# laiviet/ed-gated-gcn

Hardware: AMD Instinct MI355X
Metric: gated_gcn_forward_edges_per_sec (higher is better)
Workload: dtype f32 (fp16 MFMA + block-scaled fp8 correction MFMA, fp32 accumulate)

## Files before the change

### ed-gated-gcn_amd/csrc/capi.hip

```cpp
#include "fused_args.h"
#include <cstdlib>

#include <cstring>

namespace ggcn {

char *error_buffer()
{
    static thread_local char buf[512] = "";
    return buf;
}

int fail(int code, const char *fmt, ...)
{
    va_list ap;
    va_start(ap, fmt);
    vsnprintf(error_buffer(), 512, fmt, ap);
    va_end(ap);
    return code;
}

namespace {
constexpr int kMaxRangeFlagReaders = 16;
struct RangeFlagReaders {
// ... 415 lines not shown
    const char *form = getenv("GGCN_BLOCK_FORM");
    return (block8_shape(B, T, K, F) && !(form && form[0] == '4')) ? 8 : 4;
}

int ggcn_linear_form(int entry, const void *X, int64_t ldx, const void *W, int64_t ldw, const void *Y, int64_t ldy, int64_t M, int K,
                     int F, int precision)
{
    const char *who = "ggcn_linear_form";
    const uintptr_t xa = reinterpret_cast<uintptr_t>(X), ya = reinterpret_cast<uintptr_t>(Y);
    auto split = [&](int x_bytes, bool y_f32) -> int {
        if (linear_split_grid(M, F) > (int64_t)INT32_MAX) return -fail(GGCN_EUNSUPPORTED, "%s: M too large", who);
        return linear_split_form(x_bytes, y_f32, X, ldx, Y, ldy, K, F);
    };
    switch (entry) {
        case GGCN_ENTRY_LINEAR:
            if (int rc = linear_entry_checks(who, !X || !Y, M, K, F, ldx, ldy)) return -rc;
            if (precision == GGCN_PREC_BF16X3 || precision == GGCN_PREC_F16MX8) return split(4, true);
            if (precision != GGCN_PREC_FP32) return -fail(GGCN_EINVAL, "%s: ggcn_linear has no precision %d", who, precision);
            if (!W) return -fail(GGCN_EINVAL, "%s: ggcn_linear(fp32): W is NULL", who);
            if (ldw < F) return -fail(GGCN_EINVAL, "%s: ggcn_linear(fp32): ldw < F", who);
            return linear_fp32_form(X, ldx, W, ldw, K, F);
        case GGCN_ENTRY_LINEAR_H:
            if (precision != GGCN_PREC_BF16X3 && precision != GGCN_PREC_F16MX8 && precision != GGCN_PREC_F16)
                return -fail(GGCN_EUNSUPPORTED, "%s: ggcn_linear_h has no precision %d", who, precision);
            if (int rc = linear_entry_checks(who, !X || !Y, M, K, F, ldx, ldy)) return -rc;
            if (precision != GGCN_PREC_F16) return split(2, false);
            if (linear_split_grid(M, F) > (int64_t)INT32_MAX) return -fail(GGCN_EUNSUPPORTED, "%s: M too large", who);
            return linear_f16_form(X, ldx, K);
        case GGCN_ENTRY_LINEAR_BF16:
        case GGCN_ENTRY_LINEAR_OUT_BF16: {
            const bool out = entry == GGCN_ENTRY_LINEAR_OUT_BF16;
            if (int rc = linear_entry_checks(who, !X || !Y, M, K, F, ldx, ldy)) return -rc;
            if (xa % (out ? 4 : 2) || ya % (out ? 2 : 4)) return -fail(GGCN_EINVAL, "%s: X / Y not aligned to their element size", who);
            return split(out ? 4 : 2, !out);
        }
        case GGCN_ENTRY_LINEAR_SCALED:
            if (!X || !Y) return -fail(GGCN_EINVAL, "%s: null pointer", who);
            if (M <= 0 || K <= 0 || F <= 0 || ldx < K || ldy < F) return -fail(GGCN_EINVAL, "%s: M=%lld K=%d F=%d", who, (long long)M, K, F);
            if (!linear_scaled_takes(static_cast<const float *>(X), ldx, static_cast<const float *>(Y), ldy, K, F))
                return -fail(GGCN_EUNSUPPORTED, "%s: ggcn_linear_scaled needs K %% 32 == 0, F %% 4 == 0 and 16-byte aligned rows", who);
            return split(4, true);
        default:
            return -fail(GGCN_EINVAL, "%s: unknown entry %d", who, entry);
    }
}

int ggcn_lab_block_fused8(const float *X, int64_t ldx, const void *wpack1, const void *wpack12, const void *graph_ops,
                          const void *graph_ops2, const float *bias1, const float *bias_mid, const float *bias2, int B, int T, int K, int F,
                          const float *gate1, const float *gate2, float *x_out, int64_t ld2, float *x1, float *y1, float *pool_out,
                          float *overlap_partial, uint64_t *stamps, ggcn_stream_t stream)
{
    const int flags = (getenv("GGCN_LAB_BLOCK8_ROWMAJOR") ? kBlock8RowMajor : 0) | (getenv("GGCN_LAB_BLOCK8_NODMA") ? kBlock8NoDma : 0) |
                      (getenv("GGCN_LAB_BLOCK8_SAMESLOTS") ? kBlock8SameSlots : 0) |
                      (getenv("GGCN_LAB_BLOCK8_PRIO") ? kBlock8Prio : 0);
    FusedArgs a = {};
    a.X = X; a.ldx = ldx; a.graph_ops = bytes(graph_ops); a.graph_ops2 = bytes(graph_ops2);
    a.stamps = reinterpret_cast<unsigned long long *>(stamps);
    a.B = B; a.T = T; a.K = K; a.F = F; a.n_parts = 2;
    LayerPart &l1 = a.part[0], &l2 = a.part[1];
    l1.wpack = bytes(wpack1); l1.bias = bias1; l1.pool_gate_a = gate1; l1.pool_gate_b = gate2;
    l1.pool_a = x1; l1.pool_b = y1; l1.ov_partial = overlap_partial;
    l2.wpack = bytes(wpack12); l2.bias = bias2; l2.mid = bias_mid; l2.store_gate = gate2; l2.pool_gate_a = gate2;
    l2.out = x_out; l2.ldo = (int)(ld2 < 0 ? -1 : ld2 > (int64_t)INT32_MAX ? (int64_t)INT32_MAX : ld2); l2.pool_a = pool_out;
    return block_fused8("ggcn_lab_block_fused8", a, flags, as_stream(stream));
}

int ggcn_gate_pool_backward_weighted(const float *out, int64_t ldo, const float *store_gate, const float *gate_a, const float *gate_b,
                                     const float *d_out, int64_t ldd, const float *d_pa, const float *d_pb, const void *graph_ops_wt,
                                     const float *inv, int B, int T, int F, float *dH, int64_t ldh, float *dY, int64_t ldy, float *d_sg,
                                     float *d_ga, float *d_gb, float *d_bsum, ggcn_stream_t stream)
{
    return gate_pool_backward_weighted(out, ldo, store_gate, gate_a, gate_b, d_out, ldd, d_pa, d_pb, graph_ops_wt, inv, B, T, F, dH, ldh,
                                       dY, ldy, d_sg, d_ga, d_gb, d_bsum, as_stream(stream));
}

int ggcn_layer_fused_drop(const float *X, int64_t ldx, const void *wpack, const uint32_t *rowmask, const void *graph_ops,
                          const float *bias, int B, int T, int K, int F, const float *store_gate,
                          const float *pool_gate_a, const float *pool_gate_b, float *out, int64_t ldo,
                          float *pool_a, float *pool_b, int precision, float p, uint64_t seed, int sel_store,
                          int sel_a, int sel_b, ggcn_stream_t stream)
{
    const char *who = "ggcn_layer_fused";
    FusedArgs a = {};
    if (int rc = entry_drop_spec("ggcn_layer_fused_drop", p, seed, sel_store, sel_a, sel_b, a.drop)) return rc;
    if (int rc = layer_entry_checks(who, out, ldo, nullptr, nullptr)) return rc;
    a.X = X; a.ldx = ldx; a.rowmask = rowmask; a.graph_ops = bytes(graph_ops);
    a.B = B; a.T = T; a.K = K; a.F = F; a.n_parts = 1;
    LayerPart &l = a.part[0];
    l.wpack = bytes(wpack); l.bias = bias; l.store_gate = store_gate; l.pool_gate_a = pool_gate_a; l.pool_gate_b = pool_gate_b;
    l.out = out; l.ldo = (int)ldo; l.pool_a = pool_a; l.pool_b = pool_b;
    return launch_fused(who, a, precision, as_stream(stream));
}

size_t ggcn_dweight_workspace_bytes(int64_t n_rows, int K, int F, int precision)
{
    return precision == GGCN_PREC_FP32 ? dweight_workspace_bytes(n_rows, K, F) : dweight_bx3_workspace_bytes(n_rows, K, F);
}

int ggcn_dweight(const float *X, int64_t ldx, const float *dH, int64_t ldg, int64_t n_rows, int K, int F,
                 float *dW, int64_t lddw, int precision, void *workspace, ggcn_stream_t stream)
{
    if (precision == GGCN_PREC_FP32)
        return dweight(X, ldx, dH, ldg, n_rows, K, F, dW, lddw, workspace, as_stream(stream));
    if (precision != GGCN_PREC_BF16X3)
        return fail(GGCN_EUNSUPPORTED, "ggcn_dweight: precision %d (gradients need fp32 range: use bf16x3 or fp32)", precision);
    return dweight_bx3(X, ldx, dH, ldg, n_rows, K, F, dW, lddw, workspace, as_stream(stream));
}
// ... 50 lines not shown
```

### ed-gated-gcn_amd/csrc/f16mx8_core.h

```cpp
#pragma once
#include "bf16x3_core.h"

namespace ggcn {
namespace mx8 {

using namespace bx3;

typedef _Float16 f16x8 __attribute__((ext_vector_type(8)));
typedef int i32x8 __attribute__((ext_vector_type(8)));
typedef int i32x4 __attribute__((ext_vector_type(4)));

#ifndef GGCN_WH8_STORED
#define GGCN_WH8_STORED 0
#endif
constexpr int kWh8Bytes = GGCN_WH8_STORED ? 64 * 16 : 0;
constexpr int kOffWl8 = 2 * 1024, kOffWh8 = kOffWl8 + 64 * 16, kOffScales = kOffWh8 + kWh8Bytes;
constexpr int STAGE_PACK_BYTES = kOffScales + 64 * 4;
constexpr int XL_SHIFT = 11;
constexpr int SCALE_XL = 127 - XL_SHIFT, SCALE_XH = 127;

static __device__ unsigned int g_range_flag;
constexpr float kWindow = 448.0f;
constexpr float kHalfMax = 65504.0f;
__device__ __forceinline__ void range_verdict(float amax, float hb_scale = 0.0f, float hb_add = 0.0f, bool window = true)
// ... 38 lines not shown
    typedef float f2 __attribute__((ext_vector_type(2)));
    typedef short s2 __attribute__((ext_vector_type(2)));
    const h2 p0 = __builtin_convertvector(f2{x0, x1}, h2);
    const h2 p1 = __builtin_convertvector(f2{x2, x3}, h2);
    float r0, r1, r2, r3;
    asm("v_fma_mix_f32 %0, %1, -1.0, %2 op_sel_hi:[1,0,0]" : "=v"(r0) : "v"(p0), "v"(x0));
    asm("v_fma_mix_f32 %0, %1, -1.0, %2 op_sel:[1,0,0] op_sel_hi:[1,0,0]" : "=v"(r1) : "v"(p0), "v"(x1));
    asm("v_fma_mix_f32 %0, %1, -1.0, %2 op_sel_hi:[1,0,0]" : "=v"(r2) : "v"(p1), "v"(x2));
    asm("v_fma_mix_f32 %0, %1, -1.0, %2 op_sel:[1,0,0] op_sel_hi:[1,0,0]" : "=v"(r3) : "v"(p1), "v"(x3));
    constexpr float inv = 1.0f / (float)(1 << XL_SHIFT);
    s2 q = __builtin_bit_cast(s2, undef_vgpr());
    q = __builtin_amdgcn_cvt_scalef32_pk_fp8_f32(q, r0, r1, inv, false);
    q = __builtin_amdgcn_cvt_scalef32_pk_fp8_f32(q, r2, r3, inv, true);
    amax = amax3(x2, x3, amax3(x0, x1, amax));
    int h8 = __builtin_amdgcn_cvt_pk_fp8_f32(x0, x1, undef_vgpr(), false);
    h8 = __builtin_amdgcn_cvt_pk_fp8_f32(x2, x3, h8, true);
    Split4 o;
    o.h01 = __builtin_bit_cast(uint32_t, p0);
    o.h23 = __builtin_bit_cast(uint32_t, p1);
    o.l8 = __builtin_bit_cast(int, q);
    o.h8 = h8;
    return o;
}

__device__ __forceinline__ void set_cvt_saturate(bool on) { __builtin_amdgcn_s_setreg(1 | (23 << 6), on ? 1 : 0); }

__device__ __forceinline__ int q_lds_off(int row, int chunk)
{
    return row * ROWB + ((chunk ^ ((row >> 2) & 3) ^ (((row >> 1) & 1) << 1)) << 4);
}

#define GGCN_SB() __builtin_amdgcn_sched_barrier(0)

template <typename AT>
struct BufX {
    const AT *base;
    uint32_t bytes;
    uint32_t off[Geom<AT>::NP];
};
template <typename AT>
__device__ __forceinline__ BufX<AT> make_bufx(const AT *X, int64_t ldx, int64_t base_row, int64_t total_rows,
                                              const int (&rel)[Geom<AT>::NP], int tid)
{
    BufX<AT> b;
    const int64_t left = (total_rows - base_row) * ldx * (int64_t)sizeof(AT);
    b.base = X + base_row * ldx;
    b.bytes = (uint32_t)(left < 0x7fffffff ? left : 0x7fffffff);
#pragma unroll
    for (int i = 0; i < Geom<AT>::NP; ++i)
        b.off[i] = rel[i] < 0 ? 0x80000000u
                              : (uint32_t)(((int64_t)rel[i] * ldx + (tid % Geom<AT>::TPR) * Geom<AT>::EPT) * (int64_t)sizeof(AT));
    return b;
}
template <typename AT, bool AVEC, bool KFULL, bool ZROWS, bool RBLK = false, bool BUF = false, int NB = 4, bool XS = false, int XP = 4, int SLOT0 = 0>
__device__ __forceinline__ void mainloop(const AT *const (&arow)[Geom<AT>::NP], const bool (&avalid)[Geom<AT>::NP],
                                         const char *__restrict__ wpack, int K, int stages_packed, int wm,
                                         int nt0, int n_tiles_total, char *lds, f32x16 (&acc)[4][RN], int rot = 0, int nblk = 4,
                                         float *amax_out = nullptr, const BufX<AT> *bufx = nullptr, float xscale = 1.0f, int pass0 = 0)
{
    static_assert(!BUF || (AVEC && KFULL && sizeof(AT) == 4), "buffer loads: whole 16-byte pieces of fp32 rows");
    static_assert(NB >= 1 && NB <= 4 && (NB == 4 || (sizeof(AT) == 4 && !RBLK)), "NB < 4: fp32 rows (pass i = block i), no run-time count");
    constexpr int NPL0 = Geom<AT>::NP < NB ? Geom<AT>::NP : NB;
    constexpr int NPL = NPL0 < XP ? NPL0 : XP;
    static_assert(XP == 4 || (sizeof(AT) == 4 && NB == 4 && !RBLK), "XP < 4: fp32 rows, whole tiles");
    static_assert(SLOT0 >= 0 && SLOT0 + XP <= 4, "the staging passes sit behind the stage's four row-block slots");
    using G = Geom<AT>;
    constexpr int EPT = G::EPT, NP = G::NP, NQ = EPT / 4;
    static_assert(BK == 32 && NP <= 4 && RN == 2, "the slot schedule below is written for BK = 32, <= 4 passes, RN = 2");
    const int tid = threadIdx.x & (kThreads - 1);
    const int lane = tid & 63;
    const int s_k = (tid % G::TPR) * EPT;

    set_cvt_saturate(true);
    float amax = 0.0f;

    constexpr int kRsrcFlags = 0x00020000;
    __amdgpu_buffer_rsrc_t xr, wr;
    if constexpr (BUF) {
        xr = __builtin_amdgcn_make_buffer_rsrc(const_cast<AT *>(bufx->base), 0, (int)bufx->bytes, kRsrcFlags);
        wr = __builtin_amdgcn_make_buffer_rsrc(const_cast<char *>(wpack), 0, 0x7fffffff, kRsrcFlags);
    }
    float ra[NP][EPT];
    auto load_a_pass = [&](int i, int k0) {
        const int gk = k0 + s_k;
        if constexpr (BUF) {
            const float4 t = __builtin_bit_cast(float4, __builtin_amdgcn_raw_buffer_load_b128(xr, bufx->off[i], k0 * (int)sizeof(AT), 0));
            ra[i][0] = t.x; ra[i][1] = t.y; ra[i][2] = t.z; ra[i][3] = t.w;
        } else if constexpr (AVEC) {
            load16<AT>(arow[i] + ((KFULL || gk < K) ? gk : 0), ra[i]);
        } else {
#pragma unroll
            for (int c = 0; c < EPT; ++c) ra[i][c] = elem_to_float(arow[i][(gk + c < K) ? gk + c : 0]);
        }
    };
    Split4 sp[NQ];
    auto split_pass = [&](int i, int k0) {
        const int gk = k0 + s_k;
#pragma unroll
        for (int q = 0; q < NQ; ++q) {
            float x[4];
#pragma unroll
            for (int c = 0; c < 4; ++c) {
                x[c] = ra[i][4 * q + c];
                if constexpr (!KFULL || ZROWS) {
                    bool in = true;
                    if constexpr (!KFULL) in = gk + 4 * q + c < K;
                    if constexpr (ZROWS && !BUF) in = in && avalid[i];
                    x[c] = in ? x[c] : 0.0f;
                }
                if constexpr (XS) x[c] *= xscale;
            }
            sp[q] = split4(x[0], x[1], x[2], x[3], amax);
        }
    };
    auto write_pass = [&](int buf, int i) {
        char *h_plane = lds + buf * (2 * BM * ROWB);
        char *q_plane = h_plane + BM * ROWB;
        const int row = stage_row<AT>(XP == 4 ? i : i + pass0);
#pragma unroll
        for (int q = 0; q < NQ; ++q) {
            const int kq = s_k + 4 * q;
            *reinterpret_cast<uint2 *>(h_plane + a_lds_off(row, kq >> 3) + (kq & 4) * 2) = make_uint2(sp[q].h01, sp[q].h23);
// ... 57 lines not shown
    auto wh8_of = [&](const f16x8 &f0, const f16x8 &f1, int sc) -> i32x4 {
        typedef _Float16 h2 __attribute__((ext_vector_type(2)));
        typedef short s2 __attribute__((ext_vector_type(2)));
        const float inv = __builtin_bit_cast(float, (sc & 0xff00) << 15);
        i32x4 o;
#pragma unroll
        for (int d = 0; d < 4; ++d) {
            const f16x8 &f = d < 2 ? f0 : f1;
            const int e = (d & 1) * 4;
            s2 q = __builtin_bit_cast(s2, undef_vgpr());
            q = __builtin_amdgcn_cvt_scalef32_pk_fp8_f16(q, h2{f[e], f[e + 1]}, inv, false);
            q = __builtin_amdgcn_cvt_scalef32_pk_fp8_f16(q, h2{f[e + 2], f[e + 3]}, inv, true);
            o[d] = __builtin_bit_cast(int, q);
        }
        return o;
    };

    const int f_row = wm * 128 + (lane & 31);
    const int f_half = lane >> 5;
    const int scale_a = f_half ? SCALE_XH : SCALE_XL;
    auto read_h = [&](int buf, int i, f16x8 (&a)[2]) {
        const char *h_plane = lds + buf * (2 * BM * ROWB);
        const int row = f_row + i * 32;
        a[0] = *reinterpret_cast<const f16x8 *>(h_plane + a_lds_off(row, f_half));
        a[1] = *reinterpret_cast<const f16x8 *>(h_plane + a_lds_off(row, 2 + f_half));
    };
    auto read_q = [&](int buf, int i, i32x8 &a) {
        const char *q_plane = lds + buf * (2 * BM * ROWB) + BM * ROWB;
        const int row = f_row + i * 32;
        const i32x4 lo = *reinterpret_cast<const i32x4 *>(q_plane + q_lds_off(row, f_half));
        const i32x4 hi = *reinterpret_cast<const i32x4 *>(q_plane + q_lds_off(row, 2 + f_half));
        a = __builtin_shufflevector(lo, hi, 0, 1, 2, 3, 4, 5, 6, 7);
    };

#pragma unroll
    for (int i = 0; i < 4; ++i)
#pragma unroll
        for (int j = 0; j < RN; ++j)
#pragma unroll
            for (int r = 0; r < 16; ++r) acc[i][j][r] = 0.0f;

    f16x8 b0[RN], b1[RN];
    i32x4 bq[RN];
    i32x4 bw[RN];
    int sq[RN];
    const int stages = (K + BK - 1) / BK;

    auto kstage = [&](int n) {
        n = n < stages ? n : stages - 1;
        const int s = n + rot;
        return s >= stages ? s - stages : s;
    };
#pragma unroll
    for (int p = 0; p < NPL; ++p) load_a_pass(p, kstage(0) * BK);
    load_bf(kstage(0), b0, b1);
#pragma unroll
    for (int p = 0; p < NPL; ++p) {
        split_pass(p, kstage(0) * BK);
        write_pass(0, p);
    }
#pragma unroll
    for (int p = 0; p < NPL; ++p) load_a_pass(p, kstage(1) * BK);
    __syncthreads();

    auto stage = [&](int st, auto bufc) {
        constexpr int buf = decltype(bufc)::value;
        const int k_next1 = kstage(st + 1) * BK;
        const int ka = kstage(st + 2) * BK;
        f16x8 ah[2][2];
        i32x8 aq[2];
        read_h(buf, 0, ah[0]);
        load_bq(kstage(st), bq, sq);
        if constexpr (GGCN_WH8_STORED) load_wh8(kstage(st), bw);
        GGCN_SB();
#pragma unroll
        for (int i = 0; i < NB; ++i) {
            const bool stages_here = i - SLOT0 >= 0 && i - SLOT0 < NP && i - SLOT0 < XP;
            if (i < NB - 1) read_h(buf, i + 1, ah[(i + 1) & 1]);
            else read_q(buf, 0, aq[0]);
            GGCN_SB();
            if (!RBLK || i < nblk) acc[i][0] = __builtin_amdgcn_mfma_f32_32x32x16_f16(ah[i & 1][0], b0[0], acc[i][0], 0, 0, 0);
            GGCN_SB();
            if (stages_here) split_pass(i - SLOT0, k_next1);
            GGCN_SB();
            if (!RBLK || i < nblk) acc[i][1] = __builtin_amdgcn_mfma_f32_32x32x16_f16(ah[i & 1][0], b0[1], acc[i][1], 0, 0, 0);
            GGCN_SB();
            if (stages_here) write_pass(buf ^ 1, i - SLOT0);
            GGCN_SB();
            if (!RBLK || i < nblk) acc[i][0] = __builtin_amdgcn_mfma_f32_32x32x16_f16(ah[i & 1][1], b1[0], acc[i][0], 0, 0, 0);
            GGCN_SB();
            if (stages_here) load_a_pass(i - SLOT0, ka);
            GGCN_SB();
            if (!RBLK || i < nblk) acc[i][1] = __builtin_amdgcn_mfma_f32_32x32x16_f16(ah[i & 1][1], b1[1], acc[i][1], 0, 0, 0);
            GGCN_SB();
        }
        i32x8 bm[RN];
#pragma unroll
        for (int j = 0; j < RN; ++j) {
            i32x4 w;
            if constexpr (GGCN_WH8_STORED) w = bw[j];
            else w = wh8_of(b0[j], b1[j], sq[j]);
            bm[j] = i32x8{w[0], w[1], w[2], w[3], bq[j][0], bq[j][1], bq[j][2], bq[j][3]};
        }
        GGCN_SB();
#pragma unroll
        for (int i = 0; i < NB; ++i) {
            if (i < NB - 1) read_q(buf, i + 1, aq[(i + 1) & 1]);
// ... 25 lines not shown
```

### ed-gated-gcn_amd/csrc/fused_args.h

```cpp
#pragma once
#include "common.h"
#include "dropout_hash.h"

namespace ggcn {

struct LayerPart {
    const char *wpack;
    const float *bias;
    const float *mid;
    const float *pre;
    const float *store_gate;
    const float *pool_gate_a;
    const float *pool_gate_b;
    float *out;
    float *pool_a, *pool_b;
    float *ov_partial;
    int ldo;
};

struct FusedArgs {
    const float *X;
    int64_t ldx;
    const uint32_t *rowmask;
    const char *graph_ops;
    const char *graph_ops2;
    const float *ov_in;
    float *ov_out;
    int B, T, K, F;
    int g_tiles, n_wg, n_parts, k_steps;
    LayerPart part[2];
    DropSpec drop;
    unsigned long long *stamps;
    const __bf16 *Xb;
};

inline bool vector_row_stores(const FusedArgs &a, const LayerPart &lp)
{
    return (a.F % 4 == 0) && (lp.ldo % 4 == 0) && aligned16(lp.out) && (int64_t)a.T * lp.ldo * 4 < ((int64_t)1 << 31);
}

int fused_part_checks(const char *who, const FusedArgs &a, bool &vst);

int launch_fused(const char *who, FusedArgs &a, int precision, hipStream_t st, bool weighted_block = false);

int launch_fused_weighted_wide(const char *who, FusedArgs &a, int precision, hipStream_t st);

enum BlockKind { kBlockBinary, kBlockWeighted, kBlockBf16 };
int launch_block(const char *who, FusedArgs &a, BlockKind kind, int precision, hipStream_t st);

constexpr int kBlock8RowMajor = 1, kBlock8NoDma = 2, kBlock8SameSlots = 4, kBlock8Prio = 8;
bool block8_shape(int B, int T, int K, int F);
bool block8_takes(const FusedArgs &a);
int block_fused8(const char *who, FusedArgs &a, int flags, hipStream_t st);

}
```

### ed-gated-gcn_amd/csrc/fused_block8.hip

```cpp
#include "fused_common.h"

#include <cstdlib>

namespace ggcn {
namespace {

constexpr int kB8Threads = 512;
constexpr int kB8Lds = kLdsBytes + 2 * kEpiLdsBytes;

__device__ __forceinline__ bool getenv_slot_same(const FusedArgs &a) { return (a.k_steps & 0x20000000) != 0; }

template <int BASE>
__device__ __forceinline__ float staged_mid_max(const char *lds, bool dma, int lane)
{
    if (dma) {
        const float4 m4 = *reinterpret_cast<const float4 *>(lds + EpiLds<BASE>::kBias + BN * 4 + lane * 16);
        float mm = fmaxf(fmaxf(fabsf(m4.x), fabsf(m4.y)), fmaxf(fabsf(m4.z), fabsf(m4.w)));
#pragma unroll
        for (int d = 32; d >= 1; d >>= 1) mm = fmaxf(mm, __shfl_xor(mm, d));
        return mm;
    }
    const float4 mm = *reinterpret_cast<const float4 *>(lds + EpiLds<BASE>::kMidMax);
    return fmaxf(fmaxf(mm.x, mm.y), fmaxf(mm.z, mm.w));
}

template <bool FULLT, bool VST>
__global__ __launch_bounds__(kB8Threads, 1) void block_fused8_kernel(const FusedArgs a)
{
    extern __shared__ __attribute__((aligned(16))) char lds[];
    const int B = a.B, T = a.T, K = a.K, F = a.F;
    int n_wgi, g_tile;
    if (a.n_parts == 2) {
        const int xcd = blockIdx.x & 7, qb = blockIdx.x >> 3;
        const int total = a.g_tiles * a.n_wg, per_xcd = (total + 7) >> 3;
        const int w = xcd * per_xcd + qb;
        if (qb >= per_xcd || w >= total) return;
        n_wgi = w / a.g_tiles;
        g_tile = w - n_wgi * a.g_tiles;
    } else {
        if (!tile_of_block(blockIdx.x, a.g_tiles, a.n_wg, g_tile, n_wgi)) return;
    }

    const int tid8 = threadIdx.x;
    const unsigned long long t_start = a.stamps ? __builtin_amdgcn_s_memrealtime() : 0;
    const int group = __builtin_amdgcn_readfirstlane(tid8 >> 8);
    const int tid = tid8 & 255;
    const int wave = __builtin_amdgcn_readfirstlane(tid >> 6);
    const LayerPart &lp = a.part[group];
    const int gt0 = g_tile * 4, g0 = gt0;
    const int n_tiles_total = (F + NT - 1) / NT;
    const int nt0 = n_wgi * (BN / NT) + wave * RN;

    constexpr int NP = Geom<float>::NP;
    const float *arow[NP];
    bool avalid[NP];
    int rel[NP];
#pragma unroll
    for (int i = 0; i < NP; ++i) {
        const int row = stage_row<float>(i < 2 ? i + 2 * group : 0);
        const int g = gt0 + (row >> 5), r = row & 31;
        avalid[i] = i < 2 && (g < B) && (FULLT || r < T);
        arow[i] = a.X;
        rel[i] = avalid[i] ? (row >> 5) * T + (row & 31) : -1;
    }
    const bool dma = (a.n_wg * BN == F) && (gt0 + 4 <= B) && a.ov_in == nullptr && a.ov_out == nullptr && (a.k_steps & 0x40000000) != 0;
    const int k_steps = a.k_steps & 0x0fffffff;
    if (dma) {
        if (group == 0) stage_epilogue_operands_dma<kLdsBytes>(a, lp, g0, n_wgi, lds, tid);
        else stage_epilogue_operands_dma<kLdsBytes + kEpiLdsBytes>(a, lp, g0, n_wgi, lds, tid);
    } else {
        if (group == 0) stage_epilogue_operands<kLdsBytes>(a, lp, g0, n_wgi, lds, tid);
        else stage_epilogue_operands<kLdsBytes + kEpiLdsBytes>(a, lp, g0, n_wgi, lds, tid);
    }

    f32x16 acc[4][RN];
    float amax;
    const int64_t pack_bytes = (int64_t)n_tiles_total * (k_steps / 2) * mx8::STAGE_PACK_BYTES;
    const float bw1 = *reinterpret_cast<const float *>(a.part[0].wpack + pack_bytes);
    const float bw12 = *reinterpret_cast<const float *>(a.part[1].wpack + pack_bytes);
    const unsigned long long t_loop0 = a.stamps ? __builtin_amdgcn_s_memrealtime() : 0;
    mx8::BufX<float> bx = mx8::make_bufx<float>(a.X, a.ldx, (int64_t)gt0 * T, (int64_t)B * T, rel, tid);
    if (group == 1 && (a.k_steps & 0x10000000) != 0) __builtin_amdgcn_s_setprio(1);
    if (group == 0 || getenv_slot_same(a))
        mx8::mainloop<float, true, true, !FULLT, false, true, 4, false, 2, 0>(arow, avalid, lp.wpack, K, k_steps / 2, 0, nt0, n_tiles_total, lds, acc, 0, 4,
                                                                               &amax, &bx, 1.0f, 2 * group);
    else
        mx8::mainloop<float, true, true, !FULLT, false, true, 4, false, 2, 2>(arow, avalid, lp.wpack, K, k_steps / 2, 0, nt0, n_tiles_total, lds, acc, 0, 4,
                                                                               &amax, &bx, 1.0f, 2 * group);
    unsigned long long t_loop1 = 0;
    if (a.stamps) { asm volatile("" :: "v"(acc[3][RN - 1][15])); t_loop1 = __builtin_amdgcn_s_memrealtime(); }
    mx8::range_verdict(amax, bw12, staged_mid_max<kLdsBytes + kEpiLdsBytes>(lds, dma, tid & 63), true);
    mx8::range_verdict(amax, bw1, 0.0f, false);
    if (group == 0) {
        epilogue<1, FULLT, VST, false, false, kLdsBytes>(a, lp, acc, g0, nt0, n_tiles_total, lds, tid);
    } else {
        if (lp.out) epilogue<1, FULLT, VST, true, true, kLdsBytes + kEpiLdsBytes>(a, lp, acc, g0, nt0, n_tiles_total, lds, tid);
        else epilogue<1, FULLT, VST, true, false, kLdsBytes + kEpiLdsBytes>(a, lp, acc, g0, nt0, n_tiles_total, lds, tid);
    }
    if (a.stamps && tid == 0) {
        unsigned long long *o = a.stamps + ((size_t)blockIdx.x * 2 + group) * 4;
        o[0] = t_start; o[1] = t_loop0; o[2] = t_loop1; o[3] = __builtin_amdgcn_s_memrealtime();
    }
}

}

int device_cu_count()
{
    static int cus = 0;
    if (cus == 0) {
        int dev = 0, n = 0;
        if (hipGetDevice(&dev) != hipSuccess || hipDeviceGetAttribute(&n, hipDeviceAttributeMultiprocessorCount, dev) != hipSuccess || n <= 0) n = 256;
        cus = n;
    }
    return cus;
}
bool block8_shape(int B, int T, int K, int F)
{
    if (B <= 0 || T > 32 || T <= 0 || F <= 0 || K <= 0 || F % BN != 0 || K % BK != 0) return false;
    const int64_t total = (int64_t)((B + 3) / 4) * (F / BN), cus = device_cu_count();
    return total >= 6 * cus || (total >= 3 * cus && total % cus == 0);
}
static bool block8_fast_x(const FusedArgs &a)
{
    return (a.K % BK == 0) && (a.ldx % 4 == 0) && aligned16(a.X) && (int64_t)a.ldx * 4 * 257 < ((int64_t)1 << 31);
}
static bool block8_dma_aligned(const FusedArgs &a)
{
    const LayerPart &l1 = a.part[0], &l2 = a.part[1];
    return aligned16(l1.pool_gate_a) && aligned16(l2.store_gate) && aligned16(l1.bias) && aligned16(l2.bias) && aligned16(l2.mid) &&
           aligned16(a.graph_ops) && aligned16(a.graph_ops2);
}
bool block8_takes(const FusedArgs &a)
{
    const LayerPart &l1 = a.part[0], &l2 = a.part[1];
    if (!block8_shape(a.B, a.T, a.K, a.F)) return false;
    if (!a.X || !l1.wpack || !l2.wpack || a.ldx < a.K || !aligned16(l1.wpack) || !aligned16(l2.wpack) || (l2.out && l2.ldo < a.F)) return false;
    if (!block8_fast_x(a)) return false;
    if (!a.graph_ops || !a.graph_ops2 || !l1.pool_gate_a || !l2.store_gate || !l2.mid) return false;
    if (!block8_dma_aligned(a)) return false;
    if (l2.out && !vector_row_stores(a, l2)) return false;
    return true;
}

template <typename KERN>
static bool block8_reserve_lds(KERN kern)
{
    static bool done[64] = {};
    int dev = 0;
    if (hipGetDevice(&dev) != hipSuccess) return false;
    if (dev >= 0 && dev < 64 && done[dev]) return true;
    if (hipFuncSetAttribute(reinterpret_cast<const void *>(kern), hipFuncAttributeMaxDynamicSharedMemorySize, kB8Lds) != hipSuccess) return false;
    if (dev >= 0 && dev < 64) done[dev] = true;
    return true;
}

int block_fused8(const char *who, FusedArgs &a, int flags, hipStream_t st)
{
    LayerPart &l1 = a.part[0], &l2 = a.part[1];
    if (!a.X || !l1.wpack || !l2.wpack || !a.graph_ops || !a.graph_ops2 || !l1.pool_gate_a || !l2.store_gate || !l1.pool_a || !l1.pool_b || !l2.mid)
        return fail(GGCN_EINVAL, "%s: null pointer", who);
    if (a.B <= 0 || a.T <= 0 || a.T > 32 || a.K <= 0 || a.F <= 0)
        return fail(GGCN_EUNSUPPORTED, "%s: B=%d T=%d K=%d F=%d (graphs of <= 32 nodes)", who, a.B, a.T, a.K, a.F);
    if (!l2.out && !l2.pool_a) return fail(GGCN_EINVAL, "%s: neither x nor its pool requested", who);
    if (l2.out && l2.ldo >= a.F && !vector_row_stores(a, l2)) return fail(GGCN_EUNSUPPORTED, "%s: x needs F %% 4 == 0 and 16-byte aligned rows", who);
    l1.out = nullptr; l1.ldo = 0;
    bool vst;
    if (int rc = fused_part_checks(who, a, vst)) return rc;
    if (!block8_fast_x(a)) return fail(GGCN_EUNSUPPORTED, "%s: fast shapes only (K %% 32 == 0, 16-byte aligned rows)", who);
    const bool rowmajor = (flags & kBlock8RowMajor) != 0;
    a.n_parts = rowmajor ? 3 : 2;
    a.k_steps = round_up(a.K, BK) / KSTEP;
    if ((a.F % 4 == 0) && block8_dma_aligned(a) && !(flags & kBlock8NoDma)) a.k_steps |= 0x40000000;
    if (flags & kBlock8SameSlots) a.k_steps |= 0x20000000;
    if (flags & kBlock8Prio) a.k_steps |= 0x10000000;
    a.n_wg = (a.F + BN - 1) / BN;
    const bool fullt = (a.T == 32) && (a.B % 4 == 0);
    const int64_t g_tiles = ((int64_t)a.B + 3) / 4, total = g_tiles * a.n_wg;
    const int64_t grid = rowmajor ? grid_for(g_tiles, a.n_wg) : 8 * ((total + 7) / 8);
    if (grid > (int64_t)INT32_MAX) return fail(GGCN_EUNSUPPORTED, "%s: batch too large", who);
    a.g_tiles = (int)g_tiles;
#define GGCN_L8(FT, VS)                                                                                                           \
    do {                                                                                                                          \
        auto kern = block_fused8_kernel<FT, VS>;                                                                                  \
        if (!block8_reserve_lds(kern)) return fail(GGCN_ELAUNCH, "%s: cannot reserve %d bytes of LDS", who, kB8Lds);              \
        hipLaunchKernelGGL(kern, dim3((unsigned)grid), dim3(kB8Threads), kB8Lds, st, a);                                          \
    } while (0)
    if (fullt && vst) GGCN_L8(true, true);
    else if (fullt) GGCN_L8(true, false);
    else if (vst) GGCN_L8(false, true);
    else GGCN_L8(false, false);
#undef GGCN_L8
    return check_launch(who);
}

GGCN_RANGE_FLAG_TU(range_flag_block8)

}
```

### ed-gated-gcn_amd/csrc/fused_layer.hip

```cpp
#include "fused_common.h"

#include <cstdlib>

namespace ggcn {
namespace {

__global__ __launch_bounds__(256) void graph_operands_kernel(const uint32_t *__restrict__ rowmask, int B, int T,
                                                             char *__restrict__ ops)
{
    const int lane = threadIdx.x & 63;
    const int g = blockIdx.x * 4 + (threadIdx.x >> 6);
    if (g >= B) return;
    const int r = lane & 31, h = lane >> 5;
    const uint32_t m = r < T ? rowmask[(int64_t)g * T + r] : 0u;
    char *blk = ops + (int64_t)g * kOpsBytes;
#pragma unroll
    for (int s = 0; s < 2; ++s) {
        uint32_t w[4];
#pragma unroll
        for (int q = 0; q < 4; ++q) {
            const int b = 16 * s + 8 * (q >> 1) + 2 * (q & 1) + 4 * h;
            const uint32_t two = (m >> b) & 3u;
            w[q] = (two & 1u) * 0xFFFFu + (two >> 1) * 0xFFFF0000u;
        }
// ... 367 lines not shown
    }
    if (a.drop.thr != 0 && a.part[0].mid) {
        if (a.stamps || a.ov_in || a.part[0].ov_partial) return fail(GGCN_EUNSUPPORTED, "%s: no stamps and no overlap operands under gate dropout", who);
        return launch_fused_weighted_drop(who, a, precision, avec, kfull, fullt, vst, grid, st);
    }
    if (weighted_block) return launch_fused_block_weighted(who, a, precision, avec, kfull, fullt, vst, grid, st);
#define GGCN_LAUNCH(SC, AV, KF, FT, VS) \
    hipLaunchKernelGGL((layer_fused_kernel<SC, AV, KF, FT, VS>), dim3((unsigned)grid), dim3(kThreads), 0, st, a)
#define GGCN_PICK(SC)                                                                 \
    do {                                                                              \
        if (avec && kfull && fullt && vst) GGCN_LAUNCH(SC, true, true, true, true);   \
        else if (avec && kfull && fullt) GGCN_LAUNCH(SC, true, true, true, false);    \
        else if (avec && kfull && vst) GGCN_LAUNCH(SC, true, true, false, true);      \
        else if (avec && kfull) GGCN_LAUNCH(SC, true, true, false, false);            \
        else if (avec) GGCN_LAUNCH(SC, true, false, false, false);                    \
        else GGCN_LAUNCH(SC, false, false, false, false);                             \
    } while (0)
    if (a.stamps) {
        if (!(precision == GGCN_PREC_F16MX8 && avec && kfull && fullt && vst))
            return fail(GGCN_EUNSUPPORTED, "%s: the stamped form takes f16mx8, T = 32, B %% 4 == 0, K %% 32 == 0, 16-byte rows", who);
        hipLaunchKernelGGL((layer_fused_kernel<1, true, true, true, true, true>), dim3((unsigned)grid), dim3(kThreads), 0, st, a);
    } else if (precision == GGCN_PREC_F16MX8) GGCN_PICK(1);
    else GGCN_PICK(0);
#undef GGCN_PICK
#undef GGCN_LAUNCH
    return check_launch(who);
}

int launch_block(const char *who, FusedArgs &a, BlockKind kind, int precision, hipStream_t st)
{
    const LayerPart &first = a.part[0], &second = a.part[1];
    if (kind == kBlockWeighted && a.T > 32) return fail(GGCN_EUNSUPPORTED, "%s: T=%d > 32 (one weighted layer launch per layer)", who, a.T);
    if (kind == kBlockWeighted && precision == GGCN_PREC_F16MX6) return fail(GGCN_EUNSUPPORTED, "%s: bf16x3 or f16mx8", who);
    if (kind == kBlockBf16 && a.T > 32)
        return fail(GGCN_EUNSUPPORTED, "%s: T=%d > 32 (one ggcn_layer_fused_bf16_wide per layer up to %d nodes)", who, a.T, GGCN_MASK_MAX_T);
    if (!second.store_gate) return fail(GGCN_EINVAL, "%s: gate2 is required", who);
    const bool layer1 = first.pool_a || first.pool_b || first.out || first.ov_partial;
    if (layer1 && (!first.pool_a || !first.pool_b || !first.pool_gate_a))
        return fail(GGCN_EINVAL, "%s: layer 1's outputs go together (gate1, x1 and y1; all NULL with gcn1 and overlap_partial = the eval form)", who);
    if (!second.out && !second.pool_a) return fail(GGCN_EINVAL, "%s: neither x nor its pool requested", who);
    if (kind != kBlockBinary && (!second.wpack || (layer1 && !first.wpack))) return fail(GGCN_EINVAL, "%s: null weight image", who);
    const bool ops2_ok = a.graph_ops2 && aligned16(a.graph_ops2);
    if (kind == kBlockBinary && !ops2_ok)
        return fail(GGCN_EINVAL, "%s: graph_ops2 (ggcn_graph_operands2 blocks, 16-byte aligned) is required", who);
    if (kind == kBlockWeighted && !ops2_ok)
        return fail(GGCN_EINVAL, "%s: graph_ops2w (ggcn_graph_operands2_weighted blocks, 16-byte aligned) is required", who);
    if (kind == kBlockBf16 && !a.graph_ops2) return fail(GGCN_EINVAL, "%s: graph_ops2 (the ggcn_graph_operands2 blocks of plane 0) is required", who);
    if (kind == kBlockBf16 && !ops2_ok) return fail(GGCN_EINVAL, "%s: graph_ops2 must be 16-byte aligned", who);
    if (kind == kBlockWeighted && layer1 && (!a.graph_ops || !aligned16(a.graph_ops)))
        return fail(GGCN_EINVAL, "%s: layer 1 needs graph_opsw (ggcn_graph_operands_weighted blocks, 16-byte aligned)", who);
    if (kind == kBlockBf16 && layer1 && !a.graph_ops) return fail(GGCN_EINVAL, "%s: layer 1 needs the per-graph operand blocks of ggcn_graph_operands", who);
    if (kind == kBlockBinary && layer1 && !first.out && !a.stamps && precision == GGCN_PREC_F16MX8 && block8_takes(a)) {
        const char *form = getenv("GGCN_BLOCK_FORM");
        if (!(form && form[0] == '4')) return block_fused8(who, a, kBlock8RowMajor | kBlock8Prio, st);
    }
    if (!second.mid) return fail(GGCN_EINVAL, "%s: bias_mid (W2^T.b1, zeros when gc1 has no bias) is required", who);
    if (kind == kBlockWeighted && layer1 && (!first.mid || !aligned16(first.mid)))
        return fail(GGCN_EINVAL, "%s: zero_mid ([F] zeros, 16-byte aligned) is required", who);
    if (!layer1) {
        if (a.stamps) return fail(GGCN_EUNSUPPORTED, "ggcn_debug_block_fused_stamped: the eval form is not stamped");
        if (kind == kBlockWeighted || !a.graph_ops) a.graph_ops = a.graph_ops2;
        a.part[0] = second;
        a.part[1] = LayerPart{};
        a.n_parts = 1;
    }
    return launch_fused(who, a, precision, st, kind == kBlockWeighted);
}

__global__ __launch_bounds__(256) void dropout_mask_kernel(int64_t n, int F, DropSpec d, int sel, float *__restrict__ out)
{
    const int64_t i = (int64_t)blockIdx.x * 256 + threadIdx.x;
    if (i < n) out[i] = drop_keep(drop_hash((uint32_t)i, d.seed_lo, d.seed_hi), sel, d.thr, d.scale);
}

GGCN_RANGE_FLAG_TU(range_flag_fused)

}

using namespace ggcn;

extern "C" {

int ggcn_csr_rowmask(const int32_t *rowptr, const int32_t *colidx, int B, int T, uint32_t *rowmask, ggcn_stream_t stream)
{
    const hipStream_t st = as_stream(stream);
    if (!rowptr || !colidx || !rowmask) return fail(GGCN_EINVAL, "ggcn_csr_rowmask: null pointer");
    if (B <= 0 || T <= 0) return fail(GGCN_EINVAL, "ggcn_csr_rowmask: B=%d T=%d must be positive", B, T);
    if (T > GGCN_MASK_MAX_T)
        return fail(GGCN_EUNSUPPORTED, "ggcn_csr_rowmask: T=%d > %d (row masks cover graphs of at most %d nodes)", T, GGCN_MASK_MAX_T, GGCN_MASK_MAX_T);
    const int64_t n = (int64_t)B * T;
    hipLaunchKernelGGL(rowmask_kernel, dim3((unsigned)((n + 255) / 256)), dim3(256), 0, st, rowptr, colidx, n, T,
                       rowmask);
    return check_launch("ggcn_csr_rowmask");
}

int ggcn_dropout_mask(int64_t rows, int F, float p, uint64_t seed, int sel, float *out, ggcn_stream_t stream)
{
    const hipStream_t st = as_stream(stream);
    if (!out) return fail(GGCN_EINVAL, "ggcn_dropout_mask: null pointer");
    if (rows <= 0 || F <= 0 || sel < 0 || sel > 2 || !(p >= 0.0f && p < 1.0f))
        return fail(GGCN_EINVAL, "ggcn_dropout_mask: rows=%lld F=%d sel=%d p=%g", (long long)rows, F, sel, (double)p);
    const int64_t n = rows * F;
    if (n >= ((int64_t)1 << 32)) return fail(GGCN_EUNSUPPORTED, "ggcn_dropout_mask: rows*F must fit 32 bits");
    const DropSpec d = make_drop_spec(p, seed, 0, 0, 0);
    hipLaunchKernelGGL(dropout_mask_kernel, dim3((unsigned)((n + 255) / 256)), dim3(256), 0, st, n, F, d, sel, out);
    return check_launch("ggcn_dropout_mask");
}
// ... 55 lines not shown
```

Before: 850.2 million.

## Make block8 kernel persistent and prefetch next tile's first X stage during epilogue

The fused block8 kernel becomes persistent: the grid is capped at the resident CU count and each workgroup loops over tiles with a stride, instead of launching one workgroup per tile. While the current tile runs its epilogue, the first stage of the next tile's X rows is loaded into registers through buffer loads and handed to the mainloop. This is meant to hide the X-load latency at the start of each tile and to cut workgroup launch and setup cost. In exchange it adds a __syncthreads between tiles, extra registers for the prefetched data, and possible load imbalance from the capped grid. The old one-tile-per-workgroup form can be chosen with GGCN_BLOCK_FORM=8t.

After: 856.0 million (median of 6 runs). About the same (+0.7%).

```diff
diff --git a/ed-gated-gcn_amd/csrc/capi.hip b/ed-gated-gcn_amd/csrc/capi.hip
--- a/ed-gated-gcn_amd/csrc/capi.hip
+++ b/ed-gated-gcn_amd/csrc/capi.hip
@@ -491,7 +491,8 @@
 {
     const int flags = (getenv("GGCN_LAB_BLOCK8_ROWMAJOR") ? kBlock8RowMajor : 0) | (getenv("GGCN_LAB_BLOCK8_NODMA") ? kBlock8NoDma : 0) |
                       (getenv("GGCN_LAB_BLOCK8_SAMESLOTS") ? kBlock8SameSlots : 0) |
-                      (getenv("GGCN_LAB_BLOCK8_PRIO") ? kBlock8Prio : 0);
+                      (getenv("GGCN_LAB_BLOCK8_PRIO") ? kBlock8Prio : 0) |
+                      block8_form_flags();
     FusedArgs a = {};
     a.X = X; a.ldx = ldx; a.graph_ops = bytes(graph_ops); a.graph_ops2 = bytes(graph_ops2);
     a.stamps = reinterpret_cast<unsigned long long *>(stamps);
diff --git a/ed-gated-gcn_amd/csrc/f16mx8_core.h b/ed-gated-gcn_amd/csrc/f16mx8_core.h
--- a/ed-gated-gcn_amd/csrc/f16mx8_core.h
+++ b/ed-gated-gcn_amd/csrc/f16mx8_core.h
@@ -114,13 +114,23 @@
                               : (uint32_t)(((int64_t)rel[i] * ldx + (tid % Geom<AT>::TPR) * Geom<AT>::EPT) * (int64_t)sizeof(AT));
     return b;
 }
-template <typename AT, bool AVEC, bool KFULL, bool ZROWS, bool RBLK = false, bool BUF = false, int NB = 4, bool XS = false, int XP = 4, int SLOT0 = 0>
+template <int XP>
+__device__ __forceinline__ void load_first_stage(const BufX<float> &b, float4 (&pre)[XP])
+{
+    const __amdgpu_buffer_rsrc_t xr = __builtin_amdgcn_make_buffer_rsrc(const_cast<float *>(b.base), 0, (int)b.bytes, 0x00020000);
+#pragma unroll
+    for (int p = 0; p < XP; ++p) pre[p] = __builtin_bit_cast(float4, __builtin_amdgcn_raw_buffer_load_b128(xr, b.off[p], 0, 0));
+}
+template <typename AT, bool AVEC, bool KFULL, bool ZROWS, bool RBLK = false, bool BUF = false, int NB = 4, bool XS = false, int XP = 4, int SLOT0 = 0,
+          bool PRE = false>
 __device__ __forceinline__ void mainloop(const AT *const (&arow)[Geom<AT>::NP], const bool (&avalid)[Geom<AT>::NP],
                                          const char *__restrict__ wpack, int K, int stages_packed, int wm,
                                          int nt0, int n_tiles_total, char *lds, f32x16 (&acc)[4][RN], int rot = 0, int nblk = 4,
-                                         float *amax_out = nullptr, const BufX<AT> *bufx = nullptr, float xscale = 1.0f, int pass0 = 0)
+                                         float *amax_out = nullptr, const BufX<AT> *bufx = nullptr, float xscale = 1.0f, int pass0 = 0,
+                                         const float4 *pre = nullptr)
 {
     static_assert(!BUF || (AVEC && KFULL && sizeof(AT) == 4), "buffer loads: whole 16-byte pieces of fp32 rows");
+    static_assert(!PRE || BUF, "a preloaded first stage comes through the buffer path");
     static_assert(NB >= 1 && NB <= 4 && (NB == 4 || (sizeof(AT) == 4 && !RBLK)), "NB < 4: fp32 rows (pass i = block i), no run-time count");
     constexpr int NPL0 = Geom<AT>::NP < NB ? Geom<AT>::NP : NB;
     constexpr int NPL = NPL0 < XP ? NPL0 : XP;
@@ -129,7 +139,8 @@
     using G = Geom<AT>;
     constexpr int EPT = G::EPT, NP = G::NP, NQ = EPT / 4;
     static_assert(BK == 32 && NP <= 4 && RN == 2, "the slot schedule below is written for BK = 32, <= 4 passes, RN = 2");
-    const int tid = threadIdx.x & (kThreads - 1);
+    int tid = threadIdx.x & (kThreads - 1);
+    if constexpr (PRE) asm volatile("" : "+v"(tid));
     const int lane = tid & 63;
     const int s_k = (tid % G::TPR) * EPT;
 
@@ -293,7 +304,10 @@
         return s >= stages ? s - stages : s;
     };
 #pragma unroll
-    for (int p = 0; p < NPL; ++p) load_a_pass(p, kstage(0) * BK);
+    for (int p = 0; p < NPL; ++p) {
+        if constexpr (PRE) { ra[p][0] = pre[p].x; ra[p][1] = pre[p].y; ra[p][2] = pre[p].z; ra[p][3] = pre[p].w; }
+        else load_a_pass(p, kstage(0) * BK);
+    }
     load_bf(kstage(0), b0, b1);
 #pragma unroll
     for (int p = 0; p < NPL; ++p) {
diff --git a/ed-gated-gcn_amd/csrc/fused_args.h b/ed-gated-gcn_amd/csrc/fused_args.h
--- a/ed-gated-gcn_amd/csrc/fused_args.h
+++ b/ed-gated-gcn_amd/csrc/fused_args.h
@@ -1,6 +1,8 @@
 #pragma once
 #include "common.h"
 #include "dropout_hash.h"
+
+#include <cstdlib>
 
 namespace ggcn {
 
@@ -48,7 +50,12 @@
 enum BlockKind { kBlockBinary, kBlockWeighted, kBlockBf16 };
 int launch_block(const char *who, FusedArgs &a, BlockKind kind, int precision, hipStream_t st);
 
-constexpr int kBlock8RowMajor = 1, kBlock8NoDma = 2, kBlock8SameSlots = 4, kBlock8Prio = 8;
+constexpr int kBlock8RowMajor = 1, kBlock8NoDma = 2, kBlock8SameSlots = 4, kBlock8Prio = 8, kBlock8PerTile = 16;
+inline int block8_form_flags()
+{
+    const char *form = getenv("GGCN_BLOCK_FORM");
+    return (form && form[0] == '8' && form[1] == 't' && form[2] == '\0') ? kBlock8PerTile : 0;
+}
 bool block8_shape(int B, int T, int K, int F);
 bool block8_takes(const FusedArgs &a);
 int block_fused8(const char *who, FusedArgs &a, int flags, hipStream_t st);
diff --git a/ed-gated-gcn_amd/csrc/fused_block8.hip b/ed-gated-gcn_amd/csrc/fused_block8.hip
--- a/ed-gated-gcn_amd/csrc/fused_block8.hip
+++ b/ed-gated-gcn_amd/csrc/fused_block8.hip
@@ -1,5 +1,6 @@
 #include "fused_common.h"
 
+#include <algorithm>
 #include <cstdlib>
 
 namespace ggcn {
@@ -7,6 +8,10 @@
 
 constexpr int kB8Threads = 512;
 constexpr int kB8Lds = kLdsBytes + 2 * kEpiLdsBytes;
+#ifndef GGCN_BLOCK8_PREFETCH
+#define GGCN_BLOCK8_PREFETCH 1
+#endif
+constexpr bool kB8Prefetch = GGCN_BLOCK8_PREFETCH != 0;
 
 __device__ __forceinline__ bool getenv_slot_same(const FusedArgs &a) { return (a.k_steps & 0x20000000) != 0; }
 
@@ -24,82 +29,110 @@
     return fmaxf(fmaxf(mm.x, mm.y), fmaxf(mm.z, mm.w));
 }
 
+__device__ __forceinline__ bool block8_tile(const FusedArgs &a, uint32_t v, int &g_tile, int &n_wgi)
+{
+    if (v > 0x7fffffffu) return false;
+    if (a.n_parts == 2) {
+        const int xcd = v & 7, qb = v >> 3;
+        const int total = a.g_tiles * a.n_wg, per_xcd = (total + 7) >> 3;
+        const int w = xcd * per_xcd + qb;
+        if (qb >= per_xcd || w >= total) return false;
+        n_wgi = w / a.g_tiles;
+        g_tile = w - n_wgi * a.g_tiles;
+        return true;
+    }
+    return tile_of_block((int)v, a.g_tiles, a.n_wg, g_tile, n_wgi);
+}
+
 template <bool FULLT, bool VST>
 __global__ __launch_bounds__(kB8Threads, 1) void block_fused8_kernel(const FusedArgs a)
 {
     extern __shared__ __attribute__((aligned(16))) char lds[];
     const int B = a.B, T = a.T, K = a.K, F = a.F;
-    int n_wgi, g_tile;
-    if (a.n_parts == 2) {
-        const int xcd = blockIdx.x & 7, qb = blockIdx.x >> 3;
-        const int total = a.g_tiles * a.n_wg, per_xcd = (total + 7) >> 3;
-        const int w = xcd * per_xcd + qb;
-        if (qb >= per_xcd || w >= total) return;
-        n_wgi = w / a.g_tiles;
-        g_tile = w - n_wgi * a.g_tiles;
-    } else {
-        if (!tile_of_block(blockIdx.x, a.g_tiles, a.n_wg, g_tile, n_wgi)) return;
-    }
+    const uint32_t stride = gridDim.x;
+    uint32_t v = blockIdx.x;
+    int g_tile, n_wgi;
+    if (!block8_tile(a, v, g_tile, n_wgi)) return;
 
     const int tid8 = threadIdx.x;
-    const unsigned long long t_start = a.stamps ? __builtin_amdgcn_s_memrealtime() : 0;
     const int group = __builtin_amdgcn_readfirstlane(tid8 >> 8);
     const int tid = tid8 & 255;
     const int wave = __builtin_amdgcn_readfirstlane(tid >> 6);
-    const LayerPart &lp = a.part[group];
-    const int gt0 = g_tile * 4, g0 = gt0;
     const int n_tiles_total = (F + NT - 1) / NT;
-    const int nt0 = n_wgi * (BN / NT) + wave * RN;
-
+    const int k_steps = a.k_steps & 0x0fffffff;
+    const int64_t pack_bytes = (int64_t)n_tiles_total * (k_steps / 2) * mx8::STAGE_PACK_BYTES;
+    const float bw1 = *reinterpret_cast<const float *>(a.part[0].wpack + pack_bytes);
+    const float bw12 = *reinterpret_cast<const float *>(a.part[1].wpack + pack_bytes);
+    if (group == 1 && (a.k_steps & 0x10000000) != 0) __builtin_amdgcn_s_setprio(1);
     constexpr int NP = Geom<float>::NP;
     const float *arow[NP];
     bool avalid[NP];
-    int rel[NP];
 #pragma unroll
-    for (int i = 0; i < NP; ++i) {
-        const int row = stage_row<float>(i < 2 ? i + 2 * group : 0);
-        const int g = gt0 + (row >> 5), r = row & 31;
-        avalid[i] = i < 2 && (g < B) && (FULLT || r < T);
-        arow[i] = a.X;
-        rel[i] = avalid[i] ? (row >> 5) * T + (row & 31) : -1;
-    }
-    const bool dma = (a.n_wg * BN == F) && (gt0 + 4 <= B) && a.ov_in == nullptr && a.ov_out == nullptr && (a.k_steps & 0x40000000) != 0;
-    const int k_steps = a.k_steps & 0x0fffffff;
-    if (dma) {
-        if (group == 0) stage_epilogue_operands_dma<kLdsBytes>(a, lp, g0, n_wgi, lds, tid);
-        else stage_epilogue_operands_dma<kLdsBytes + kEpiLdsBytes>(a, lp, g0, n_wgi, lds, tid);
-    } else {
-        if (group == 0) stage_epilogue_operands<kLdsBytes>(a, lp, g0, n_wgi, lds, tid);
-        else stage_epilogue_operands<kLdsBytes + kEpiLdsBytes>(a, lp, g0, n_wgi, lds, tid);
-    }
-
-    f32x16 acc[4][RN];
-    float amax;
-    const int64_t pack_bytes = (int64_t)n_tiles_total * (k_steps / 2) * mx8::STAGE_PACK_BYTES;
-    const float bw1 = *reinterpret_cast<const float *>(a.part[0].wpack + pack_bytes);
-    const float bw12 = *reinterpret_cast<const float *>(a.part[1].wpack + pack_bytes);
-    const unsigned long long t_loop0 = a.stamps ? __builtin_amdgcn_s_memrealtime() : 0;
-    mx8::BufX<float> bx = mx8::make_bufx<float>(a.X, a.ldx, (int64_t)gt0 * T, (int64_t)B * T, rel, tid);
-    if (group == 1 && (a.k_steps & 0x10000000) != 0) __builtin_amdgcn_s_setprio(1);
-    if (group == 0 || getenv_slot_same(a))
-        mx8::mainloop<float, true, true, !FULLT, false, true, 4, false, 2, 0>(arow, avalid, lp.wpack, K, k_steps / 2, 0, nt0, n_tiles_total, lds, acc, 0, 4,
-                                                                               &amax, &bx, 1.0f, 2 * group);
-    else
-        mx8::mainloop<float, true, true, !FULLT, false, true, 4, false, 2, 2>(arow, avalid, lp.wpack, K, k_steps / 2, 0, nt0, n_tiles_total, lds, acc, 0, 4,
-                                                                               &amax, &bx, 1.0f, 2 * group);
-    unsigned long long t_loop1 = 0;
-    if (a.stamps) { asm volatile("" :: "v"(acc[3][RN - 1][15])); t_loop1 = __builtin_amdgcn_s_memrealtime(); }
-    mx8::range_verdict(amax, bw12, staged_mid_max<kLdsBytes + kEpiLdsBytes>(lds, dma, tid & 63), true);
-    mx8::range_verdict(amax, bw1, 0.0f, false);
-    if (group == 0) {
-        epilogue<1, FULLT, VST, false, false, kLdsBytes>(a, lp, acc, g0, nt0, n_tiles_total, lds, tid);
-    } else {
-        if (lp.out) epilogue<1, FULLT, VST, true, true, kLdsBytes + kEpiLdsBytes>(a, lp, acc, g0, nt0, n_tiles_total, lds, tid);
-        else epilogue<1, FULLT, VST, true, false, kLdsBytes + kEpiLdsBytes>(a, lp, acc, g0, nt0, n_tiles_total, lds, tid);
-    }
-    if (a.stamps && tid == 0) {
-        unsigned long long *o = a.stamps + ((size_t)blockIdx.x * 2 + group) * 4;
-        o[0] = t_start; o[1] = t_loop0; o[2] = t_loop1; o[3] = __builtin_amdgcn_s_memrealtime();
+    for (int i = 0; i < NP; ++i) { arow[i] = a.X; avalid[i] = i < 2; }
+    auto tile_bufx = [&](bool have, int gt0) {
+        int rel[NP];
+#pragma unroll
+        for (int i = 0; i < NP; ++i) {
+            const int row = stage_row<float>(i < 2 ? i + 2 * group : 0);
+            const int g = gt0 + (row >> 5), r = row & 31;
+            rel[i] = (have && i < 2 && (g < B) && (FULLT || r < T)) ? (row >> 5) * T + r : -1;
+        }
+        return mx8::make_bufx<float>(a.X, a.ldx, have ? (int64_t)gt0 * T : (int64_t)B * T, (int64_t)B * T, rel, tid);
+    };
+    float4 pre[2];
+    if constexpr (kB8Prefetch) mx8::load_first_stage<2>(tile_bufx(true, g_tile * 4), pre);
+
+    for (;;) {
+        const unsigned long long t_start = a.stamps ? __builtin_amdgcn_s_memrealtime() : 0;
+        int tid_m = tid, group_m = group;
+        asm volatile("" : "+v"(tid_m), "+s"(group_m));
+        const LayerPart &lp_m = a.part[group_m];
+        const int gt0 = g_tile * 4, g0 = gt0;
+        const int nt0 = n_wgi * (BN / NT) + wave * RN;
+        const bool dma = (a.n_wg * BN == F) && (gt0 + 4 <= B) && a.ov_in == nullptr && a.ov_out == nullptr && (a.k_steps & 0x40000000) != 0;
+        if (dma) {
+            if (group_m == 0) stage_epilogue_operands_dma<kLdsBytes>(a, lp_m, g0, n_wgi, lds, tid_m);
+            else stage_epilogue_operands_dma<kLdsBytes + kEpiLdsBytes>(a, lp_m, g0, n_wgi, lds, tid_m);
+        } else {
+            if (group_m == 0) stage_epilogue_operands<kLdsBytes>(a, lp_m, g0, n_wgi, lds, tid_m);
+            else stage_epilogue_operands<kLdsBytes + kEpiLdsBytes>(a, lp_m, g0, n_wgi, lds, tid_m);
+        }
+
+        f32x16 acc[4][RN];
+        float amax;
+        const unsigned long long t_loop0 = a.stamps ? __builtin_amdgcn_s_memrealtime() : 0;
+        const mx8::BufX<float> bx = tile_bufx(true, gt0);
+        if (group_m == 0 || getenv_slot_same(a))
+            mx8::mainloop<float, true, true, !FULLT, false, true, 4, false, 2, 0, kB8Prefetch>(arow, avalid, lp_m.wpack, K, k_steps / 2, 0, nt0, n_tiles_total, lds,
+                                                                                                acc, 0, 4, &amax, &bx, 1.0f, 2 * group_m, pre);
+        else
+            mx8::mainloop<float, true, true, !FULLT, false, true, 4, false, 2, 2, kB8Prefetch>(arow, avalid, lp_m.wpack, K, k_steps / 2, 0, nt0, n_tiles_total, lds,
+                                                                                                acc, 0, 4, &amax, &bx, 1.0f, 2 * group_m, pre);
+        unsigned long long t_loop1 = 0;
+        if (a.stamps) { asm volatile("" :: "v"(acc[3][RN - 1][15])); t_loop1 = __builtin_amdgcn_s_memrealtime(); }
+        mx8::range_verdict(amax, bw12, staged_mid_max<kLdsBytes + kEpiLdsBytes>(lds, dma, tid_m & 63), true);
+        mx8::range_verdict(amax, bw1, 0.0f, false);
+        int tid_e = tid, group_e = group;
+        asm volatile("" : "+v"(tid_e), "+s"(group_e));
+        const LayerPart &lp_e = a.part[group_e];
+        int g_next = 0, n_next = 0;
+        const bool more = block8_tile(a, v + stride, g_next, n_next);
+        if constexpr (kB8Prefetch) mx8::load_first_stage<2>(tile_bufx(more, g_next * 4), pre);
+        if (group_e == 0) {
+            epilogue<1, FULLT, VST, false, false, kLdsBytes>(a, lp_e, acc, g0, nt0, n_tiles_total, lds, tid_e);
+        } else {
+            if (lp_e.out) epilogue<1, FULLT, VST, true, true, kLdsBytes + kEpiLdsBytes>(a, lp_e, acc, g0, nt0, n_tiles_total, lds, tid_e);
+            else epilogue<1, FULLT, VST, true, false, kLdsBytes + kEpiLdsBytes>(a, lp_e, acc, g0, nt0, n_tiles_total, lds, tid_e);
+        }
+        if (a.stamps && tid_e == 0) {
+            unsigned long long *o = a.stamps + ((size_t)v * 2 + group_e) * 4;
+            o[0] = t_start; o[1] = t_loop0; o[2] = t_loop1; o[3] = __builtin_amdgcn_s_memrealtime();
+        }
+        if (!more) break;
+        __syncthreads();
+        v += stride;
+        g_tile = g_next;
+        n_wgi = n_next;
     }
 }
 
@@ -177,8 +210,10 @@
     a.n_wg = (a.F + BN - 1) / BN;
     const bool fullt = (a.T == 32) && (a.B % 4 == 0);
     const int64_t g_tiles = ((int64_t)a.B + 3) / 4, total = g_tiles * a.n_wg;
-    const int64_t grid = rowmajor ? grid_for(g_tiles, a.n_wg) : 8 * ((total + 7) / 8);
-    if (grid > (int64_t)INT32_MAX) return fail(GGCN_EUNSUPPORTED, "%s: batch too large", who);
+    const int64_t ids = rowmajor ? grid_for(g_tiles, a.n_wg) : 8 * ((total + 7) / 8);
+    if (ids > (int64_t)INT32_MAX) return fail(GGCN_EUNSUPPORTED, "%s: batch too large", who);
+    const int64_t resident = std::max(8, device_cu_count() & ~7);
+    const int64_t grid = (flags & kBlock8PerTile) ? ids : std::min(ids, resident);
     a.g_tiles = (int)g_tiles;
 #define GGCN_L8(FT, VS)                                                                                                           \
     do {                                                                                                                          \
diff --git a/ed-gated-gcn_amd/csrc/fused_layer.hip b/ed-gated-gcn_amd/csrc/fused_layer.hip
--- a/ed-gated-gcn_amd/csrc/fused_layer.hip
+++ b/ed-gated-gcn_amd/csrc/fused_layer.hip
@@ -443,7 +443,7 @@
     if (kind == kBlockBf16 && layer1 && !a.graph_ops) return fail(GGCN_EINVAL, "%s: layer 1 needs the per-graph operand blocks of ggcn_graph_operands", who);
     if (kind == kBlockBinary && layer1 && !first.out && !a.stamps && precision == GGCN_PREC_F16MX8 && block8_takes(a)) {
         const char *form = getenv("GGCN_BLOCK_FORM");
-        if (!(form && form[0] == '4')) return block_fused8(who, a, kBlock8RowMajor | kBlock8Prio, st);
+        if (!(form && form[0] == '4')) return block_fused8(who, a, kBlock8RowMajor | kBlock8Prio | block8_form_flags(), st);
     }
     if (!second.mid) return fail(GGCN_EINVAL, "%s: bias_mid (W2^T.b1, zeros when gc1 has no bias) is required", who);
     if (kind == kBlockWeighted && layer1 && (!first.mid || !aligned16(first.mid)))
```
